# Grzetan/3D-Reconstruction-Triangulation

Hardware: NVIDIA B200
Metric: 3D points/sec (8-cam DLT, 20% missing) (higher is better)
Workload: dtype f64

## Files before the change

3d-reconstruction-triangulation_b200/csrc/tri_matrix.cu:

```cuda
#include "tri_pipe.cuh"

namespace tri {

__device__ __forceinline__ void load12(const double (&src)[12], double (&P)[12]) {
  const double2* v = reinterpret_cast<const double2*>(src);
#pragma unroll
  for (int k = 0; k < 6; k++) { const double2 q = v[k]; P[2 * k] = q.x; P[2 * k + 1] = q.y; }
}
__device__ __forceinline__ void load12(const float (&src)[12], float (&P)[12]) {
  const float4* v = reinterpret_cast<const float4*>(src);
#pragma unroll
  for (int k = 0; k < 3; k++) { const float4 q = v[k]; P[4 * k] = q.x; P[4 * k + 1] = q.y; P[4 * k + 2] = q.z; P[4 * k + 3] = q.w; }
}

template <typename T>
__device__ __forceinline__ void acc_row(T a0, T a1, T a2, T b, T (&M)[6], T (&v)[3]) {
  M[0] = fma_(a0, a0, M[0]); M[1] = fma_(a0, a1, M[1]); M[2] = fma_(a0, a2, M[2]); v[0] = fma_(a0, b, v[0]);
  M[3] = fma_(a1, a1, M[3]); M[4] = fma_(a1, a2, M[4]); v[1] = fma_(a1, b, v[1]);
  M[5] = fma_(a2, a2, M[5]); v[2] = fma_(a2, b, v[2]);
}

template <typename T>
__device__ __forceinline__ const T* absent_row(const DltRig<T>& rig, uint32_t mask, int group, int n_in_group) {
  const uint32_t absent = ~(mask >> (8 * group)) & ((1u << n_in_group) - 1u);
  return rig.absent + ((size_t)group * 256 + absent) * DLT_TABLE_ROW;
}
__device__ __forceinline__ void sub_row(const float* row, float (&M)[6], float (&v)[3]) {
  const float4* r = reinterpret_cast<const float4*>(row);
  const float4 t0 = __ldg(r), t1 = __ldg(r + 1), t2 = __ldg(r + 2);
  M[0] -= t0.x; M[1] -= t0.y; M[2] -= t0.z; M[3] -= t0.w; M[4] -= t1.x; M[5] -= t1.y; v[0] -= t1.z; v[1] -= t1.w; v[2] -= t2.x;
}

// ... 14 lines not shown
    T P[12];
    load12(rig.P[c], P);
    if constexpr (CENTRED) { x -= rig.pix0[c][0]; y -= rig.pix0[c][1]; }
    if constexpr (MASKING == MASK_TABLE) { x = valid ? x : T(0); y = valid ? y : T(0); }
#pragma unroll
    for (int r = 0; r < 2; r++) {
      const T u = r == 0 ? x : y;
      T a0 = fma_(-u, P[8], P[4 * r]), a1 = fma_(-u, P[9], P[4 * r + 1]), a2 = fma_(-u, P[10], P[4 * r + 2]);
      const T b = fma_(u, P[11], -P[4 * r + 3]);
      if constexpr (MASKING == MASK_SELECT_HI) { a0 = mask_coeff(a0, valid); a1 = mask_coeff(a1, valid); a2 = mask_coeff(a2, valid); }
      acc_row<T>(a0, a1, a2, b, a.M, a.v);
    }
  }
  static __device__ __forceinline__ void add_chunk(const Rig& rig, int c, T x, T y, bool valid, Acc& a) { add(rig, c, x, y, valid, a); }
  static __device__ __forceinline__ void solve(const Rig& rig, const Acc& a, uint32_t mask, int, T (&X)[3], int, int&) {
    Acc r = a;
    if constexpr (MASKING == MASK_TABLE)
      for (int g = 0; 8 * g < rig.n_use; g++) sub_row(absent_row<T>(rig, mask, g, min(8, rig.n_use - 8 * g)), r.M, r.v);
    solve_sym3<T>(r.M, r.v, X);
  }
  static __device__ __forceinline__ T residual(const Rig& rig, int c, T x, T y, const T (&X)[3]) {
    const T(&P)[12] = rig.P[c];
    if constexpr (CENTRED) { x -= rig.pix0[c][0]; y -= rig.pix0[c][1]; }
    const T e0 = fma_(fma_(-x, P[8], P[0]), X[0], fma_(fma_(-x, P[9], P[1]), X[1], fma_(fma_(-x, P[10], P[2]), X[2], -fma_(x, P[11], -P[3]))));
    const T e1 = fma_(fma_(-y, P[8], P[4]), X[0], fma_(fma_(-y, P[9], P[5]), X[1], fma_(fma_(-y, P[10], P[6]), X[2], -fma_(y, P[11], -P[7]))));
    return fma_(e0, e0, mul_(e1, e1));
  }
  static __device__ __forceinline__ double error(T sum, int n) { return sqrt((double)sum / (double)(2 * n)); }
  static __device__ __forceinline__ void to_world(const Rig& rig, T (&X)[3]) {
    if constexpr (CENTRED) { X[0] += rig.origin[0]; X[1] += rig.origin[1]; X[2] += rig.origin[2]; }
  }
};

struct DltTile64 {
  static constexpr int FPT = 2;
  using S = DltPolicy<double, false, MASK_SELECT_HI>;
  using Rig = DltRig<double>;
  using Real = double;
  template <int NC, int PIX, bool WIDE, class RS>
  static __device__ __forceinline__ void run(const Rig& rig, const RS& raw, int, double (&X)[2][3], uint32_t (&mask)[2],
                                             double (&err)[2], int (&iters)[2]) {
    typename S::Acc acc[2];
    mask[0] = mask[1] = 0;
#pragma unroll
    for (int c = 0; c < NC; c++) {
      double P[12];
      load12(rig.P[c], P);
      double x[2], y[2];
      bool ok[2];
      if constexpr (PIX == PIX_F32) {
        const Views<float, PIX, 2> q = decode<float, PIX, 2>(raw[c]);
#pragma unroll
        for (int j = 0; j < 2; j++) { ok[j] = q.v[j]; x[j] = (double)q.x[j]; y[j] = (double)q.y[j]; }
      } else {
        const Views<double, PIX, 2> q = decode<double, PIX, 2>(raw[c]);
#pragma unroll
        for (int j = 0; j < 2; j++) { ok[j] = q.v[j]; x[j] = q.x[j]; y[j] = q.y[j]; }
      }
#pragma unroll
      for (int j = 0; j < 2; j++) {
        mask[j] |= (ok[j] ? 1u : 0u) << c;
#pragma unroll
        for (int r = 0; r < 2; r++) {
          const double u = r == 0 ? x[j] : y[j];
          double a0 = fma_(-u, P[8], P[4 * r]), a1 = fma_(-u, P[9], P[4 * r + 1]), a2 = fma_(-u, P[10], P[4 * r + 2]);
          const double b = fma_(u, P[11], -P[4 * r + 3]);
          a0 = mask_coeff(a0, ok[j]); a1 = mask_coeff(a1, ok[j]); a2 = mask_coeff(a2, ok[j]);
          acc_row<double>(a0, a1, a2, b, acc[j].M, acc[j].v);
        }
      }
    }
#pragma unroll
    for (int j = 0; j < 2; j++) {
      X[j][0] = X[j][1] = X[j][2] = 0;
      err[j] = 0;
      iters[j] = 0;
      const int n = __popc(mask[j]);
      if (n >= 2) {
        solve_sym3<double>(acc[j].M, acc[j].v, X[j]);
        if constexpr (WIDE) {
          double e = 0;
#pragma unroll
          for (int c = 0; c < NC; c++) {
            const Views<double, PIX, 2> q = decode<double, PIX, 2>(raw[c]);
            if (q.v[j]) e += S::residual(rig, c, q.x[j], q.y[j], X[j]);
          }
          err[j] = S::error(e, n);
        }
      }
    }
  }
};

struct __align__(16) DltRigX2 {
  float2 A[TRI_MAX_CAMS][8];
  float2 N[TRI_MAX_CAMS][4];
  float2 npix0[TRI_MAX_CAMS][2];
  float origin[3];
  const float* absent;
};

struct DltX2Tile {
  static constexpr int FPT = 2;
  using Rig = DltRigX2;
  using Real = float;
  template <int NC, int PIX, bool WIDE, class RS>
  static __device__ __forceinline__ void run(const Rig& rig, const RS& raw, int, float (&X)[2][3], uint32_t (&mask)[2],
                                             double (&err)[2], int (&iters)[2]) {
    float2 M[6] = {{0, 0}, {0, 0}, {0, 0}, {0, 0}, {0, 0}, {0, 0}}, v[3] = {{0, 0}, {0, 0}, {0, 0}};
    uint32_t mask0 = 0, mask1 = 0;
#pragma unroll
    for (int c = 0; c < NC; c++) {
// ... 49 lines not shown
            if (q.v[j]) {
              const float x = q.x[j] + rig.npix0[c][0].x, y = q.y[j] + rig.npix0[c][1].x;
              const float e0 = fmaf(fmaf(x, rig.N[c][0].x, rig.A[c][0].x), Xr[j][0], fmaf(fmaf(x, rig.N[c][1].x, rig.A[c][1].x), Xr[j][1],
                               fmaf(fmaf(x, rig.N[c][2].x, rig.A[c][2].x), Xr[j][2], -fmaf(x, rig.N[c][3].x, rig.A[c][3].x))));
              const float e1 = fmaf(fmaf(y, rig.N[c][0].x, rig.A[c][4].x), Xr[j][0], fmaf(fmaf(y, rig.N[c][1].x, rig.A[c][5].x), Xr[j][1],
                               fmaf(fmaf(y, rig.N[c][2].x, rig.A[c][6].x), Xr[j][2], -fmaf(y, rig.N[c][3].x, rig.A[c][7].x))));
              e += fmaf(e0, e0, e1 * e1);
            }
          }
          err[j] = sqrt((double)e / (double)(2 * __popc(j == 0 ? mask0 : mask1)));
        }
      }
      X[j][0] = ok ? Xr[j][0] + rig.origin[0] : 0.f; X[j][1] = ok ? Xr[j][1] + rig.origin[1] : 0.f; X[j][2] = ok ? Xr[j][2] + rig.origin[2] : 0.f;
    }
  }
};


static DltRigX2 make_x2(const DltRig<float>& r) {
  DltRigX2 x;
  for (int c = 0; c < TRI_MAX_CAMS; c++) {
    const float* P = r.P[c];
    const float A[8] = {P[0], P[1], P[2], -P[3], P[4], P[5], P[6], -P[7]};
    const float N[4] = {-P[8], -P[9], -P[10], P[11]};
    for (int k = 0; k < 8; k++) x.A[c][k] = make_float2(A[k], A[k]);
    for (int k = 0; k < 4; k++) x.N[c][k] = make_float2(N[k], N[k]);
    for (int k = 0; k < 2; k++) x.npix0[c][k] = make_float2(-r.pix0[c][k], -r.pix0[c][k]);
  }
  for (int k = 0; k < 3; k++) x.origin[k] = r.origin[k];
  x.absent = r.absent;
  return x;
}

cudaError_t launch_dlt(const LaunchCtx& ctx, bool f32, int pixfmt, const DltRig<double>& rig64_,
                       const DltRig<float>& rig32_, const void* d_xy, int n_use, int64_t n_frames,
                       int64_t cam_stride, const BatchOut& out) {
  if (n_frames <= 0) return cudaSuccess;
  using P32 = DltPolicy<float, true, MASK_TABLE>;
  using P64 = DltPolicy<double, false, MASK_SELECT_HI>;
  if (f32) {
    DltRig<float> rig32 = rig32_;
    rig32.n_use = n_use;
    const DltRigX2 x2 = make_x2(rig32);
    if (pixfmt == PIX_F32) return launch_streamed<DltX2Tile, P32, PIX_F32, 2, 2, 3, true>(ctx, x2, rig32, d_xy, n_use, n_frames, cam_stride, out, 0);
    if (pixfmt == PIX_F64) return launch_streamed<DltX2Tile, P32, PIX_F64, 2, 2, 3>(ctx, x2, rig32, d_xy, n_use, n_frames, cam_stride, out, 0);
    return launch_streamed<DltX2Tile, P32, PIX_U16, 2, 2, 3>(ctx, x2, rig32, d_xy, n_use, n_frames, cam_stride, out, 0);
  }
  DltRig<double> rig64 = rig64_;
  rig64.n_use = n_use;
  if (pixfmt == PIX_F32) return launch_streamed<DltTile64, P64, PIX_F32, 2, 2, 2>(ctx, rig64, rig64, d_xy, n_use, n_frames, cam_stride, out, 0);
  if (pixfmt == PIX_F64) return launch_batch_policy<P64, PIX_F64, 1, 3>(ctx, rig64, d_xy, n_use, n_frames, cam_stride, out, 0);
  return launch_streamed<DltTile64, P64, PIX_U16, 2, 3, 2>(ctx, rig64, rig64, d_xy, n_use, n_frames, cam_stride, out, 0);
}

}
```

3d-reconstruction-triangulation_b200/csrc/tri_api.cu:

```cuda
#include <math.h>
#include <stdlib.h>
#include <string.h>

#include <algorithm>
#include <string>
#include <thread>
#include <vector>

#include "tri_engine.cuh"

namespace tri {

static thread_local std::string g_error;
void set_error(const std::string& s) { g_error = s; }
int fail(int status, const std::string& s) {
  g_error = s;
  return status;
}
int cuda_fail(cudaError_t err, const char* what) {
  g_error = std::string(what) + ": " + cudaGetErrorString(err);
  return TRI_ERR_CUDA;
}
#define TRI_CUDA(call)                                         \
  do {                                                         \
// ... 90 lines not shown
static cudaError_t upload_ray_table(RayFold<T>& f, int n_cams) {
  const std::vector<T> tab = ray_mask_table(f, n_cams);
  T* d = nullptr;
  cudaError_t err = cudaMalloc((void**)&d, tab.size() * sizeof(T));
  if (err == cudaSuccess) err = cudaMemcpy(d, tab.data(), tab.size() * sizeof(T), cudaMemcpyHostToDevice);
  f.mask_table = d;
  return err;
}

static inline float fma_h(float a, float b, float c) { return fmaf(a, b, c); }
template <typename T>
static std::vector<T> dlt_absent_table(const DltRig<T>& r, int n_cams) {
  const int groups = (n_cams + 7) / 8;
  std::vector<T> tab((size_t)groups * 256 * DLT_TABLE_ROW, (T)0);
  for (int g = 0; g < groups; g++)
    for (int m = 0; m < 256; m++) {
      T M[6] = {0, 0, 0, 0, 0, 0}, v[3] = {0, 0, 0};
      for (int k = 0; k < 8 && 8 * g + k < n_cams; k++) {
        if (!(m >> k & 1)) continue;
        const T* P = r.P[8 * g + k];
        for (int row = 0; row < 2; row++) {
          const T a0 = P[4 * row], a1 = P[4 * row + 1], a2 = P[4 * row + 2], b = -P[4 * row + 3];
          M[0] = fma_h(a0, a0, M[0]); M[1] = fma_h(a0, a1, M[1]); M[2] = fma_h(a0, a2, M[2]); v[0] = fma_h(a0, b, v[0]);
          M[3] = fma_h(a1, a1, M[3]); M[4] = fma_h(a1, a2, M[4]); v[1] = fma_h(a1, b, v[1]);
          M[5] = fma_h(a2, a2, M[5]); v[2] = fma_h(a2, b, v[2]);
        }
      }
      T* row = &tab[((size_t)g * 256 + m) * DLT_TABLE_ROW];
      for (int k = 0; k < 6; k++) row[k] = M[k];
      for (int k = 0; k < 3; k++) row[6 + k] = v[k];
    }
  return tab;
}
template <typename T>
static cudaError_t upload_dlt_table(DltRig<T>& r, int n_cams) {
  const std::vector<T> tab = dlt_absent_table(r, n_cams);
  T* d = nullptr;
  cudaError_t err = cudaMalloc((void**)&d, tab.size() * sizeof(T));
  if (err == cudaSuccess) err = cudaMemcpy(d, tab.data(), tab.size() * sizeof(T), cudaMemcpyHostToDevice);
  r.absent = d;
  return err;
}

static void build_rigs(tri_engine* e) {
  memset(&e->fold64, 0, sizeof(e->fold64));
  memset(&e->fold32, 0, sizeof(e->fold32));
  memset(&e->rig64, 0, sizeof(e->rig64));
  memset(&e->rig32, 0, sizeof(e->rig32));
  memset(&e->ray, 0, sizeof(e->ray));
  double c0[3];
  rig_centre(e, c0);
  for (int k = 0; k < 3; k++) e->rig32.origin[k] = (float)c0[k];
  for (int k = 0; k < 3; k++) c0[k] = (double)e->rig32.origin[k];
  for (int c = 0; c < e->n_cams; c++) {
    const tri_camera& cam = e->cams[c];
    for (int k = 0; k < 12; k++) e->rig64.P[c][k] = cam.P[k];
    const double px = floor(cam.width / 2.0), py = floor(cam.height / 2.0);
    double Q[12];
    for (int k = 0; k < 4; k++) {
      Q[k] = cam.P[k] - px * cam.P[8 + k];
      Q[4 + k] = cam.P[4 + k] - py * cam.P[8 + k];
      Q[8 + k] = cam.P[8 + k];
    }
    for (int r = 0; r < 3; r++) Q[r * 4 + 3] += Q[r * 4] * c0[0] + Q[r * 4 + 1] * c0[1] + Q[r * 4 + 2] * c0[2];
    for (int k = 0; k < 12; k++) e->rig32.P[c][k] = (float)Q[k];
    e->rig32.pix0[c][0] = (float)px;
    e->rig32.pix0[c][1] = (float)py;
    e->ray.aspect[c] = (double)cam.width / (double)cam.height;
    e->ray.width[c] = (double)cam.width;
// ... 157 lines not shown
int tri_version(void) { return 100; }
const char* tri_last_error(void) { return g_error.c_str(); }

int tri_device_count(void) {
  int n = 0;
  if (cudaGetDeviceCount(&n) != cudaSuccess) {
    cudaGetLastError();
    return 0;
  }
  return n;
}

int tri_create(int n_cams, const tri_camera* cams, int device, tri_engine** out) {
  if (!out) return fail(TRI_ERR_ARG, "null out pointer");
  *out = nullptr;
  if (n_cams < 1 || n_cams > TRI_MAX_CAMS || !cams) return fail(TRI_ERR_ARG, "n_cams must be in [1, TRI_MAX_CAMS]");
  int n_dev = tri_device_count();
  if (n_dev <= 0) return fail(TRI_ERR_NO_DEVICE, "no CUDA device: the engine has no CPU path");
  if (device < 0 || device >= n_dev) return fail(TRI_ERR_ARG, "device index out of range");
  for (int c = 0; c < n_cams; c++)
    if (cams[c].width <= 0 || cams[c].height <= 0) return fail(TRI_ERR_ARG, "camera width/height must be positive");
  DeviceGuard g(device);
  cudaDeviceProp prop;
  TRI_CUDA(cudaGetDeviceProperties(&prop, device));
  if (prop.major < 10) return fail(TRI_ERR_NO_DEVICE, "libtri_b200 is built for sm_100a (B200) only");
  tri_engine* e = new tri_engine();
  e->device = device;
  e->n_cams = n_cams;
  e->sm_count = prop.multiProcessorCount;
  memcpy(e->cams, cams, sizeof(tri_camera) * n_cams);
  build_rigs(e);
  cudaError_t err = cudaMalloc((void**)&e->d_first_bad, 2 * sizeof(unsigned long long));
  if (err == cudaSuccess) err = cudaMemset(e->d_first_bad, 0xff, 2 * sizeof(unsigned long long));
  if (err == cudaSuccess) err = upload_dlt_table(e->rig32, n_cams);
  if (err == cudaSuccess) err = upload_ray_table(e->fold64, n_cams);
  if (err == cudaSuccess) err = upload_ray_table(e->fold32, n_cams);
  if (err == cudaSuccess) err = cudaStreamCreateWithFlags(&e->stream, cudaStreamNonBlocking);
  for (int i = 0; i < N_SLOTS && err == cudaSuccess; i++) err = cudaStreamCreateWithFlags(&e->slots[i].stream, cudaStreamNonBlocking);
  if (err != cudaSuccess) {
    int st = cuda_fail(err, "tri_create");
    tri_destroy(e);
    return st;
  }
  *out = e;
  return TRI_OK;
}

void tri_destroy(tri_engine* e) {
  if (!e) return;
  DeviceGuard g(e->device);
  cudaDeviceSynchronize();
  for (int i = 0; i < N_SLOTS; i++) {
    if (e->slots[i].d_in) cudaFree(e->slots[i].d_in);
    if (e->slots[i].d_out) cudaFree(e->slots[i].d_out);
    if (e->slots[i].stream) cudaStreamDestroy(e->slots[i].stream);
  }
  if (e->cls_work && e->cls_work_free) e->cls_work_free(e->cls_work);
  if (e->d_scratch) cudaFree(e->d_scratch);
  if (e->stream) cudaStreamDestroy(e->stream);
  if (e->d_first_bad) cudaFree(e->d_first_bad);
  if (e->rig32.absent) cudaFree(const_cast<float*>(e->rig32.absent));
  if (e->fold64.mask_table) cudaFree(const_cast<double*>(e->fold64.mask_table));
  if (e->fold32.mask_table) cudaFree(const_cast<float*>(e->fold32.mask_table));
  delete e;
}

int tri_engine_device(const tri_engine* e) { return e ? e->device : -1; }
int tri_engine_cameras(const tri_engine* e) { return e ? e->n_cams : 0; }
int64_t tri_kernel_launches(const tri_engine* e) { return e ? e->launches : 0; }

int tri_triangulate_points_device(tri_engine* e, int mode, unsigned flags, const void* d_xy, int n_point_cams,
                                  int64_t n_frames, int64_t cam_stride, const tri_batch_out* d_out, void* stream) {
  int n_use = 0, fmt = 0;
  int st = check_batch_args(e, mode, d_xy, n_point_cams, n_frames, cam_stride, d_out, &n_use);
  if (st != TRI_OK) return st;
  if ((st = pix_format(flags, &fmt)) != TRI_OK) return st;
  if (n_frames == 0) return TRI_OK;
  DeviceGuard g(e->device);
  BatchOut out{d_out->xyz_f32, d_out->xyz_f64, d_out->mask, d_out->err, d_out->iters};
  if (n_use == 0) return too_few_device(e, n_frames, out, (cudaStream_t)stream);
  return launch_batch(e, e->ctx((cudaStream_t)stream), mode, flags, fmt, d_xy, n_use, n_frames, cam_stride, out);
}

int tri_enable_peer_access(tri_engine* e, int peer_device) {
  if (!e) return fail(TRI_ERR_ARG, "null engine");
  if (peer_device == e->device) return TRI_OK;
  DeviceGuard g(e->device);
  int can = 0;
  TRI_CUDA(cudaDeviceCanAccessPeer(&can, e->device, peer_device));
  if (!can) return fail(TRI_ERR_ARG, "no peer access between these GPUs");
  cudaError_t err = cudaDeviceEnablePeerAccess(peer_device, 0);
  if (err == cudaErrorPeerAccessAlreadyEnabled) { cudaGetLastError(); return TRI_OK; }
  if (err != cudaSuccess) return cuda_fail(err, "cudaDeviceEnablePeerAccess");
  return TRI_OK;
// ... 182 lines not shown
```

3d-reconstruction-triangulation_b200/csrc/tri_batch.cuh:

```cuda
#pragma once
#include "tri_common.cuh"

namespace tri {

constexpr int BATCH_THREADS = 256;

template <typename T>
struct View2 {
  T x0, y0, x1, y1;
  bool v0, v1;
};

template <typename T, int PIX>
__device__ __forceinline__ View2<T> fetch2(const char* row, int64_t pair) {
  View2<T> r;
  if constexpr (PIX == PIX_F32) {
    float4 q = ld_stream(reinterpret_cast<const float4*>(row) + pair);
    r.v0 = pix_valid(q.x, q.y);
    r.v1 = pix_valid(q.z, q.w);
    r.x0 = to_real<T>(q.x); r.y0 = to_real<T>(q.y); r.x1 = to_real<T>(q.z); r.y1 = to_real<T>(q.w);
  } else if constexpr (PIX == PIX_F64) {
    double2 a = ld_stream(reinterpret_cast<const double2*>(row) + 2 * pair);
    double2 b = ld_stream(reinterpret_cast<const double2*>(row) + 2 * pair + 1);
    r.v0 = pix_valid(a.x, a.y);
    r.v1 = pix_valid(b.x, b.y);
    r.x0 = (T)a.x; r.y0 = (T)a.y; r.x1 = (T)b.x; r.y1 = (T)b.y;
  } else {
    uint2 q = ld_stream(reinterpret_cast<const uint2*>(row) + pair);
    r.v0 = q.x != 0xffffffffu;
    r.v1 = q.y != 0xffffffffu;
    if constexpr (sizeof(T) == 8) {
      const double magic = 4503599627370496.0;
      r.x0 = __hiloint2double(0x43300000, (int)(q.x & 0xffffu)) - magic;
// ... 9 lines not shown

template <typename T, int PIX>
__device__ __forceinline__ void fetch1(const char* row, int64_t f, T& x, T& y, bool& v) {
  if constexpr (PIX == PIX_F32) {
    float2 q = ld_stream(reinterpret_cast<const float2*>(row) + f);
    v = pix_valid(q.x, q.y); x = (T)q.x; y = (T)q.y;
  } else if constexpr (PIX == PIX_F64) {
    double2 q = ld_stream(reinterpret_cast<const double2*>(row) + f);
    v = pix_valid(q.x, q.y); x = (T)q.x; y = (T)q.y;
  } else {
    unsigned q = ld_stream(reinterpret_cast<const unsigned*>(row) + f);
    v = q != 0xffffffffu; x = (T)(q & 0xffffu); y = (T)(q >> 16);
  }
}

template <typename T, int PIX, int FPT>
struct Views {
  T x[FPT], y[FPT];
  bool v[FPT];
};

template <typename T, int PIX, int FPT>
__device__ __forceinline__ Views<T, PIX, FPT> fetch(const char* row, int64_t group) {
  Views<T, PIX, FPT> r;
  if constexpr (FPT == 2) {
    View2<T> w = fetch2<T, PIX>(row, group);
    r.x[0] = w.x0; r.y[0] = w.y0; r.v[0] = w.v0; r.x[1] = w.x1; r.y[1] = w.y1; r.v[1] = w.v1;
  } else {
    fetch1<T, PIX>(row, group, r.x[0], r.y[0], r.v[0]);
  }
  return r;
}

template <class S, int NC, int PIX, int FPT, int MINB>
__global__ void __launch_bounds__(BATCH_THREADS, MINB)
batch_kernel(const __grid_constant__ typename S::Rig rig, const char* __restrict__ xy, int64_t row_bytes,
             int64_t n_groups, int n_use, BatchOut out, int opt, unsigned long long* first_bad, int64_t frame_base) {
  using T = typename S::T;
  __shared__ __align__(16) float tile[BATCH_THREADS * 3 * FPT];
  const int64_t block_group0 = (int64_t)blockIdx.x * BATCH_THREADS;
  const int64_t group = block_group0 + threadIdx.x;
  const int nc = NC > 0 ? NC : n_use;
  T X[FPT][3];
#pragma unroll
  for (int j = 0; j < FPT; j++) X[j][0] = X[j][1] = X[j][2] = 0;

  if (group < n_groups) {
    typename S::Acc acc[FPT];
    uint32_t mask[FPT];
    T e[FPT];
    int it[FPT], n[FPT];
#pragma unroll
    for (int j = 0; j < FPT; j++) { mask[j] = 0; e[j] = 0; it[j] = 0; }
    if constexpr (NC > 0) {
      Views<T, PIX, FPT> w[NC];
#pragma unroll
      for (int c = 0; c < NC; c++) w[c] = fetch<T, PIX, FPT>(xy + c * row_bytes, group);
#pragma unroll
      for (int c = 0; c < NC; c++)
#pragma unroll
        for (int j = 0; j < FPT; j++)
          { S::add(rig, c, w[c].x[j], w[c].y[j], w[c].v[j], acc[j]); mask[j] |= (w[c].v[j] ? 1u : 0u) << c; }
#pragma unroll
      for (int j = 0; j < FPT; j++) {
        n[j] = __popc(mask[j]);
        if (n[j] >= 2) S::solve(rig, acc[j], mask[j], n[j], X[j], opt, it[j]);
      }
      if (out.err) {
#pragma unroll
        for (int c = 0; c < NC; c++)
#pragma unroll
          for (int j = 0; j < FPT; j++)
            if (w[c].v[j]) e[j] += S::residual(rig, c, w[c].x[j], w[c].y[j], X[j]);
      }
    } else {
#pragma unroll 4
      for (int c = 0; c < nc; c++) {
        Views<T, PIX, FPT> w = fetch<T, PIX, FPT>(xy + c * row_bytes, group);
#pragma unroll
        for (int j = 0; j < FPT; j++)
          { S::add(rig, c, w.x[j], w.y[j], w.v[j], acc[j]); mask[j] |= (w.v[j] ? 1u : 0u) << c; }
      }
#pragma unroll
      for (int j = 0; j < FPT; j++) {
        n[j] = __popc(mask[j]);
        if (n[j] >= 2) S::solve(rig, acc[j], mask[j], n[j], X[j], opt, it[j]);
      }
      if (out.err) {
        for (int c = 0; c < nc; c++) {
          Views<T, PIX, FPT> w = fetch<T, PIX, FPT>(xy + c * row_bytes, group);
#pragma unroll
          for (int j = 0; j < FPT; j++)
            if (w.v[j]) e[j] += S::residual(rig, c, w.x[j], w.y[j], X[j]);
        }
      }
    }
#pragma unroll
    for (int j = 0; j < FPT; j++) {
      const int64_t f = FPT * group + j;
      if (n[j] >= 2) S::to_world(rig, X[j]);
      else atomicMin(first_bad, (unsigned long long)(frame_base + f));
      if (out.xyz_f64) { double* o = out.xyz_f64 + 3 * f; o[0] = X[j][0]; o[1] = X[j][1]; o[2] = X[j][2]; }
      if (out.mask) out.mask[f] = mask[j];
      if (out.err) out.err[f] = n[j] >= 2 ? S::error(e[j], n[j]) : 0.0;
      if (out.iters) out.iters[f] = it[j];
    }
  }

  if (out.xyz_f32) {
    float* t = tile + 3 * FPT * threadIdx.x;
#pragma unroll
    for (int j = 0; j < FPT; j++) { t[3 * j] = (float)X[j][0]; t[3 * j + 1] = (float)X[j][1]; t[3 * j + 2] = (float)X[j][2]; }
    __syncthreads();
    const int64_t remaining = n_groups - block_group0;
    float* dst = out.xyz_f32 + 3 * FPT * block_group0;
    if (remaining >= BATCH_THREADS && ((uintptr_t)dst & 15) == 0) {
      float4* d4 = reinterpret_cast<float4*>(dst);
      const float4* s4 = reinterpret_cast<const float4*>(tile);
#pragma unroll
      for (int i = threadIdx.x; i < BATCH_THREADS * 3 * FPT / 4; i += BATCH_THREADS) __stcs(d4 + i, s4[i]);
    } else {
      const int cnt = (int)(remaining < BATCH_THREADS ? remaining : BATCH_THREADS) * 3 * FPT;
      for (int i = threadIdx.x; i < cnt; i += BATCH_THREADS) dst[i] = tile[i];
    }
  }
}

template <class S, int PIX>
__global__ void __launch_bounds__(BATCH_THREADS)
batch_single_kernel(const __grid_constant__ typename S::Rig rig, const char* __restrict__ xy, int64_t row_bytes,
                    int64_t f_begin, int64_t f_end, int n_use, BatchOut out, int opt, unsigned long long* first_bad,
                    int64_t frame_base) {
  using T = typename S::T;
  const int64_t f = f_begin + (int64_t)blockIdx.x * BATCH_THREADS + threadIdx.x;
  if (f >= f_end) return;
  typename S::Acc acc;
  T X[3] = {0, 0, 0}, e = 0;
  uint32_t mask = 0;
  int it = 0;
  for (int c = 0; c < n_use; c++) {
    T x, y; bool ok;
    fetch1<T, PIX>(xy + c * row_bytes, f, x, y, ok);
    { S::add(rig, c, x, y, ok, acc); mask |= (ok ? 1u : 0u) << c; }
  }
  const int n = __popc(mask);
  if (n >= 2) {
    S::solve(rig, acc, mask, n, X, opt, it);
    if (out.err)
      for (int c = 0; c < n_use; c++) {
        T x, y; bool ok;
        fetch1<T, PIX>(xy + c * row_bytes, f, x, y, ok);
        if (ok) e += S::residual(rig, c, x, y, X);
      }
    S::to_world(rig, X);
  } else {
    atomicMin(first_bad, (unsigned long long)(frame_base + f));
  }
  if (out.xyz_f32) { float* o = out.xyz_f32 + 3 * f; o[0] = (float)X[0]; o[1] = (float)X[1]; o[2] = (float)X[2]; }
  if (out.xyz_f64) { double* o = out.xyz_f64 + 3 * f; o[0] = X[0]; o[1] = X[1]; o[2] = X[2]; }
  if (out.mask) out.mask[f] = mask;
  if (out.err) out.err[f] = n >= 2 ? S::error(e, n) : 0.0;
  if (out.iters) out.iters[f] = it;
}

template <class S, int PIX, int FPT, int MINB>
static cudaError_t launch_batch_policy(const LaunchCtx& ctx, const typename S::Rig& rig, const void* d_xy, int n_use,
                                       int64_t n_frames, int64_t cam_stride, const BatchOut& out, int opt) {
  const char* xy = static_cast<const char*>(d_xy);
  const int64_t row_bytes = cam_stride * pix_bytes(PIX);
  const int64_t need = FPT * pix_bytes(PIX);
  const bool vec = FPT == 1 || (((uintptr_t)xy % need == 0) && (row_bytes % need == 0));
  const int64_t n_groups = vec ? n_frames / FPT : 0;
  if (n_groups > 0) {
    const unsigned grid = (unsigned)((n_groups + BATCH_THREADS - 1) / BATCH_THREADS);
#define TRI_CASE(N)                                                                                              \
  case N:                                                                                                        \
    batch_kernel<S, N, PIX, FPT, MINB><<<grid, BATCH_THREADS, 0, ctx.stream>>>(rig, xy, row_bytes, n_groups, n_use, \
                                                                               out, opt, ctx.d_first_bad,        \
                                                                               ctx.frame_base);                  \
    break;
// ... 21 lines not shown
```

3d-reconstruction-triangulation_b200/csrc/tri_common.cuh:

```cuda
#pragma once
#include <cuda_runtime.h>
#include <stdint.h>

#include "../../include/tri_b200.h"

namespace tri {


constexpr int DLT_TABLE_ROW = 12;
template <typename T>
struct __align__(16) DltRig {
  T P[TRI_MAX_CAMS][12];
  T pix0[TRI_MAX_CAMS][2];
  T origin[3];
  const T* absent;
  int n_use;
};

struct RayRig {
  double aspect[TRI_MAX_CAMS];
  double width[TRI_MAX_CAMS], height[TRI_MAX_CAMS];
  double depth[TRI_MAX_CAMS];
  double quat[TRI_MAX_CAMS][4];
  double pos[TRI_MAX_CAMS][3];
};

template <typename T>
struct __align__(16) RayFold {
  T U0[TRI_MAX_CAMS][3], U1[TRI_MAX_CAMS][3], U2[TRI_MAX_CAMS][3];
  T ax[TRI_MAX_CAMS], bx[TRI_MAX_CAMS], ay[TRI_MAX_CAMS], by[TRI_MAX_CAMS], dd[TRI_MAX_CAMS];
  T n4[TRI_MAX_CAMS];
  T ob[TRI_MAX_CAMS][3];
  T n4ob[TRI_MAX_CAMS][3];
  T n4ob2[TRI_MAX_CAMS];
  T origin[3];
  const T* mask_table;
};
constexpr int TRI_RAY_TABLE_CAMS = 8;

struct BatchOut {
  float* xyz_f32;
  double* xyz_f64;
  uint32_t* mask;
  double* err;
  int32_t* iters;
};

enum PixFmt { PIX_F32 = 0, PIX_F64 = 1, PIX_U16 = 2 };

__host__ __device__ inline int pix_bytes(int fmt) { return fmt == PIX_F32 ? 8 : fmt == PIX_F64 ? 16 : 4; }
// ... 79 lines not shown
```

3d-reconstruction-triangulation_b200/csrc/tri_pipe.cuh:

```cuda
#pragma once
#include <type_traits>

#include "tri_batch.cuh"

namespace tri {

__device__ __forceinline__ uint32_t smem_u32(const void* p) { return (uint32_t)__cvta_generic_to_shared(p); }

template <int PIX, int FPT> struct RawPix;
template <> struct RawPix<PIX_F32, 2> { using type = float4; };
template <> struct RawPix<PIX_F32, 1> { using type = float2; };
template <> struct RawPix<PIX_U16, 2> { using type = uint2; };
template <> struct RawPix<PIX_U16, 1> { using type = unsigned; };

template <typename T, int PIX, int FPT>
__device__ __forceinline__ Views<T, PIX, FPT> decode(const typename RawPix<PIX, FPT>::type& q) {
  Views<T, PIX, FPT> r;
  if constexpr (PIX == PIX_F32 && FPT == 2) {
    r.v[0] = pix_valid(q.x, q.y); r.v[1] = pix_valid(q.z, q.w);
    r.x[0] = to_real<T>(q.x); r.y[0] = to_real<T>(q.y); r.x[1] = to_real<T>(q.z); r.y[1] = to_real<T>(q.w);
  } else if constexpr (PIX == PIX_F32 && FPT == 1) {
    r.v[0] = pix_valid(q.x, q.y); r.x[0] = to_real<T>(q.x); r.y[0] = to_real<T>(q.y);
  } else if constexpr (PIX == PIX_U16 && FPT == 2) {
    r.v[0] = q.x != 0xffffffffu; r.v[1] = q.y != 0xffffffffu;
// ... 347 lines not shown
    cudaError_t err = cudaFuncSetAttribute(kern, cudaFuncAttributeMaxDynamicSharedMemorySize, bytes);
    if (err != cudaSuccess) return err;
    int per_sm = 1;
    err = cudaOccupancyMaxActiveBlocksPerMultiprocessor(&per_sm, kern, BATCH_THREADS, bytes);
    if (err != cudaSuccess) return err;
    const int64_t grid = std::min<int64_t>(n_tiles, (int64_t)ctx.sm_count * std::max(per_sm, 1));
    kern<<<(unsigned)grid, BATCH_THREADS, bytes, ctx.stream>>>(rig, xy, row_bytes, n_tiles, n_use, out, opt, ctx.d_first_bad, ctx.frame_base);
    return cudaGetLastError();
  };
  const cudaError_t err = wants_wide(out) ? go(chunk_kernel<S, PIX, FPT, STAGES, MINB, true>) : go(chunk_kernel<S, PIX, FPT, STAGES, MINB, false>);
  if (err != cudaSuccess) return err;
  ++*ctx.launches;
  *covered = n_tiles * TILE;
  return cudaSuccess;
}

inline BatchOut advance(const BatchOut& o, int64_t frames) {
  BatchOut r = o;
  if (r.xyz_f32) r.xyz_f32 += 3 * frames;
  if (r.xyz_f64) r.xyz_f64 += 3 * frames;
  if (r.mask) r.mask += frames;
  if (r.err) r.err += frames;
  if (r.iters) r.iters += frames;
  return r;
}


template <class TS, class S, int PIX, int FPT, int STAGES, int MINB, bool LAZY = false>
static cudaError_t launch_streamed(const LaunchCtx& ctx, const typename TS::Rig& tile_rig, const typename S::Rig& rig,
                                   const void* d_xy, int n_use, int64_t n_frames, int64_t cam_stride, const BatchOut& out, int opt) {
  int64_t covered = 0;
  if constexpr (PIX != PIX_F64) {
    cudaError_t err;
    if (S::CHUNKED && n_use > CHUNK_CAMS)
      err = launch_chunk<S, PIX, S::CHUNK_FPT, 3, 2>(ctx, rig, d_xy, n_use, n_frames, cam_stride, out, opt, &covered);
    else
      err = launch_stream<TS, PIX, STAGES, MINB, LAZY>(ctx, tile_rig, d_xy, n_use, n_frames, cam_stride, out, opt, &covered);
    if (err != cudaSuccess || covered == n_frames) return err;
  }
  LaunchCtx rest = ctx;
  rest.frame_base += covered;
  return launch_batch_policy<S, PIX, FPT, (MINB > 3 ? 3 : MINB)>(rest, rig, static_cast<const char*>(d_xy) + covered * pix_bytes(PIX), n_use,
                                                n_frames - covered, cam_stride, advance(out, covered), opt);
}

}
```

Baseline: 53.65 billion.

## Replace f32-to-f64 pixel conversion with bit-shift construction and prescaled camera rows

For f32 pixels in the f64 DLT tile, each float is turned into a double by shifting its bits directly, which yields the value scaled by 2^-896. The last projection row is prescaled by 2^896 on the host so the products come out unchanged. A max-abs check with NaN propagation catches inf/NaN inputs and falls back to a noinline path that uses ordinary conversions. The aim is to avoid the F2F conversion instructions, whose f64 throughput is limited. The risks are wrong handling of denormal pixels and an extra argument passed to launch_streamed.

```diff
diff --git a/3d-reconstruction-triangulation_b200/csrc/tri_matrix.cu b/3d-reconstruction-triangulation_b200/csrc/tri_matrix.cu
--- a/3d-reconstruction-triangulation_b200/csrc/tri_matrix.cu
+++ b/3d-reconstruction-triangulation_b200/csrc/tri_matrix.cu
@@ -1,3 +1,5 @@
+#include <cmath>
+
 #include "tri_pipe.cuh"
 
 namespace tri {
@@ -78,26 +80,53 @@
   }
 };
 
+struct DltRigTile64 {
+  DltRig<double> rig;
+  double N[TRI_MAX_CAMS][4];
+  int scaled;
+};
+
+__device__ __forceinline__ double f32_scaled(float x) {
+  const int b = __float_as_int(x);
+  return __hiloint2double((b >> 3) & (int)0x8fffffff, (int)((unsigned)b << 29));
+}
+__device__ __forceinline__ float max_abs_nan(float m, float x) {
+  float r;
+  asm("max.NaN.f32 %0, %1, %2;" : "=f"(r) : "f"(m), "f"(fabsf(x)));
+  return r;
+}
+
 struct DltTile64 {
   static constexpr int FPT = 2;
   using S = DltPolicy<double, false, MASK_SELECT_HI>;
-  using Rig = DltRig<double>;
+  using Rig = DltRigTile64;
   using Real = double;
-  template <int NC, int PIX, bool WIDE, class RS>
-  static __device__ __forceinline__ void run(const Rig& rig, const RS& raw, int, double (&X)[2][3], uint32_t (&mask)[2],
-                                             double (&err)[2], int (&iters)[2]) {
-    typename S::Acc acc[2];
-    mask[0] = mask[1] = 0;
+
+  template <int NC, int PIX, bool SCALED, class RS>
+  static __device__ __forceinline__ bool accumulate(const Rig& rt, const RS& raw, typename S::Acc (&acc)[2], uint32_t (&mask)[2]) {
+    const DltRig<double>& rig = rt.rig;
+    float big = 0.f;
+#pragma unroll
+    for (int j = 0; j < 2; j++) { acc[j] = typename S::Acc(); mask[j] = 0; }
 #pragma unroll
     for (int c = 0; c < NC; c++) {
       double P[12];
       load12(rig.P[c], P);
+      if constexpr (SCALED) { P[8] = rt.N[c][0]; P[9] = rt.N[c][1]; P[10] = rt.N[c][2]; P[11] = rt.N[c][3]; }
       double x[2], y[2];
       bool ok[2];
       if constexpr (PIX == PIX_F32) {
         const Views<float, PIX, 2> q = decode<float, PIX, 2>(raw[c]);
 #pragma unroll
-        for (int j = 0; j < 2; j++) { ok[j] = q.v[j]; x[j] = (double)q.x[j]; y[j] = (double)q.y[j]; }
+        for (int j = 0; j < 2; j++) {
+          ok[j] = q.v[j];
+          if constexpr (SCALED) {
+            x[j] = f32_scaled(q.x[j]); y[j] = f32_scaled(q.y[j]);
+            big = max_abs_nan(max_abs_nan(big, q.x[j]), q.y[j]);
+          } else {
+            x[j] = (double)q.x[j]; y[j] = (double)q.y[j];
+          }
+        }
       } else {
         const Views<double, PIX, 2> q = decode<double, PIX, 2>(raw[c]);
 #pragma unroll
@@ -115,6 +144,34 @@
           acc_row<double>(a0, a1, a2, b, acc[j].M, acc[j].v);
         }
       }
+    }
+    return !SCALED || big <= 3.402823466e38f;
+  }
+
+  struct Sums {
+    typename S::Acc acc[2];
+    uint32_t mask[2];
+  };
+  template <int NC, int PIX, class RS>
+  static __device__ __noinline__ Sums accumulate_f2f(const Rig& rt, const RS raw) {
+    Sums s;
+    accumulate<NC, PIX, false>(rt, raw, s.acc, s.mask);
+    return s;
+  }
+
+  template <int NC, int PIX, bool WIDE, class RS>
+  static __device__ __forceinline__ void run(const Rig& rt, const RS& raw, int, double (&X)[2][3], uint32_t (&mask)[2],
+                                             double (&err)[2], int (&iters)[2]) {
+    const DltRig<double>& rig = rt.rig;
+    typename S::Acc acc[2];
+    if constexpr (PIX == PIX_F32) {
+      if (!rt.scaled || !accumulate<NC, PIX, true>(rt, raw, acc, mask)) {
+        const Sums s = accumulate_f2f<NC, PIX>(rt, raw);
+#pragma unroll
+        for (int j = 0; j < 2; j++) { acc[j] = s.acc[j]; mask[j] = s.mask[j]; }
+      }
+    } else {
+      accumulate<NC, PIX, false>(rt, raw, acc, mask);
     }
 #pragma unroll
     for (int j = 0; j < 2; j++) {
@@ -239,6 +296,18 @@
   return x;
 }
 
+static DltRigTile64 make_tile64(const DltRig<double>& r) {
+  DltRigTile64 t;
+  t.rig = r;
+  t.scaled = 1;
+  for (int c = 0; c < TRI_MAX_CAMS; c++)
+    for (int k = 0; k < 4; k++) {
+      t.N[c][k] = std::ldexp(r.P[c][8 + k], 896);
+      if (!std::isfinite(t.N[c][k])) t.scaled = 0;
+    }
+  return t;
+}
+
 cudaError_t launch_dlt(const LaunchCtx& ctx, bool f32, int pixfmt, const DltRig<double>& rig64_,
                        const DltRig<float>& rig32_, const void* d_xy, int n_use, int64_t n_frames,
                        int64_t cam_stride, const BatchOut& out) {
@@ -255,9 +324,10 @@
   }
   DltRig<double> rig64 = rig64_;
   rig64.n_use = n_use;
-  if (pixfmt == PIX_F32) return launch_streamed<DltTile64, P64, PIX_F32, 2, 2, 2>(ctx, rig64, rig64, d_xy, n_use, n_frames, cam_stride, out, 0);
   if (pixfmt == PIX_F64) return launch_batch_policy<P64, PIX_F64, 1, 3>(ctx, rig64, d_xy, n_use, n_frames, cam_stride, out, 0);
-  return launch_streamed<DltTile64, P64, PIX_U16, 2, 3, 2>(ctx, rig64, rig64, d_xy, n_use, n_frames, cam_stride, out, 0);
-}
-
-}
+  const DltRigTile64 t64 = make_tile64(rig64);
+  if (pixfmt == PIX_F32) return launch_streamed<DltTile64, P64, PIX_F32, 2, 2, 2, true>(ctx, t64, rig64, d_xy, n_use, n_frames, cam_stride, out, 0);
+  return launch_streamed<DltTile64, P64, PIX_U16, 2, 3, 2>(ctx, t64, rig64, d_xy, n_use, n_frames, cam_stride, out, 0);
+}
+
+}
```

Measured after the change: 50.59 billion (median of 6 runs). 5.7% lower.

## Precompute per-camera DLT moment coefficients and mask base table for f64 path

Applied to the files above, without the earlier changes.

The f64 DLT path now expands the normal-equation accumulation algebraically. Each camera contributes a constant part, looked up from a 256-entry table indexed by the validity mask, plus terms linear in x, y and x²+y² with precomputed moment coefficients K. The per-camera projection-row arithmetic is replaced by 27 FMAs against constants held in the grid-constant rig. Invalid views are zeroed instead of masked. This cuts per-point FLOPs but enlarges the kernel parameter struct, adds a global table load per point, and may shift rounding slightly.

```diff
diff --git a/3d-reconstruction-triangulation_b200/csrc/tri_api.cu b/3d-reconstruction-triangulation_b200/csrc/tri_api.cu
--- a/3d-reconstruction-triangulation_b200/csrc/tri_api.cu
+++ b/3d-reconstruction-triangulation_b200/csrc/tri_api.cu
@@ -146,9 +146,21 @@
     }
   return tab;
 }
+static std::vector<double> dlt_base_table(const DltRig<double>& r, int n_cams) {
+  std::vector<double> tab((size_t)256 * DLT_TABLE_ROW, 0.0);
+  for (int m = 0; m < 256; m++) {
+    double* row = &tab[(size_t)m * DLT_TABLE_ROW];
+    for (int c = 0; c < 8 && c < n_cams; c++) {
+      if (!(m >> c & 1)) continue;
+      double K[DLT_MOMENTS], K0D0[9];
+      dlt_moments(r.P[c], K, K0D0);
+      for (int i = 0; i < 9; i++) row[i] += K0D0[i];
+    }
+  }
+  return tab;
+}
 template <typename T>
-static cudaError_t upload_dlt_table(DltRig<T>& r, int n_cams) {
-  const std::vector<T> tab = dlt_absent_table(r, n_cams);
+static cudaError_t upload_dlt_table(DltRig<T>& r, const std::vector<T>& tab) {
   T* d = nullptr;
   cudaError_t err = cudaMalloc((void**)&d, tab.size() * sizeof(T));
   if (err == cudaSuccess) err = cudaMemcpy(d, tab.data(), tab.size() * sizeof(T), cudaMemcpyHostToDevice);
@@ -372,7 +384,8 @@
   build_rigs(e);
   cudaError_t err = cudaMalloc((void**)&e->d_first_bad, 2 * sizeof(unsigned long long));
   if (err == cudaSuccess) err = cudaMemset(e->d_first_bad, 0xff, 2 * sizeof(unsigned long long));
-  if (err == cudaSuccess) err = upload_dlt_table(e->rig32, n_cams);
+  if (err == cudaSuccess) err = upload_dlt_table(e->rig32, dlt_absent_table(e->rig32, n_cams));
+  if (err == cudaSuccess) err = upload_dlt_table(e->rig64, dlt_base_table(e->rig64, n_cams));
   if (err == cudaSuccess) err = upload_ray_table(e->fold64, n_cams);
   if (err == cudaSuccess) err = upload_ray_table(e->fold32, n_cams);
   if (err == cudaSuccess) err = cudaStreamCreateWithFlags(&e->stream, cudaStreamNonBlocking);
@@ -400,6 +413,7 @@
   if (e->stream) cudaStreamDestroy(e->stream);
   if (e->d_first_bad) cudaFree(e->d_first_bad);
   if (e->rig32.absent) cudaFree(const_cast<float*>(e->rig32.absent));
+  if (e->rig64.absent) cudaFree(const_cast<double*>(e->rig64.absent));
   if (e->fold64.mask_table) cudaFree(const_cast<double*>(e->fold64.mask_table));
   if (e->fold32.mask_table) cudaFree(const_cast<float*>(e->fold32.mask_table));
   delete e;
diff --git a/3d-reconstruction-triangulation_b200/csrc/tri_batch.cuh b/3d-reconstruction-triangulation_b200/csrc/tri_batch.cuh
--- a/3d-reconstruction-triangulation_b200/csrc/tri_batch.cuh
+++ b/3d-reconstruction-triangulation_b200/csrc/tri_batch.cuh
@@ -1,4 +1,6 @@
 #pragma once
+#include <type_traits>
+
 #include "tri_common.cuh"
 
 namespace tri {
@@ -74,6 +76,28 @@
   return r;
 }
 
+template <class S, class = void>
+struct HasBegin { static constexpr bool value = false; };
+template <class S>
+struct HasBegin<S, std::void_t<decltype(S::BEGIN)>> { static constexpr bool value = S::BEGIN; };
+
+template <class S, int PIX, int FPT>
+__device__ __forceinline__ void begin_views(const typename S::Rig& rig, const char* xy, int64_t row_bytes, int64_t group, int nc,
+                                            typename S::Acc (&acc)[FPT]) {
+  if constexpr (HasBegin<S>::value) {
+    uint32_t bits[FPT];
+#pragma unroll
+    for (int j = 0; j < FPT; j++) bits[j] = 0;
+    for (int c = 0; c < nc; c++) {
+      const Views<typename S::T, PIX, FPT> w = fetch<typename S::T, PIX, FPT>(xy + c * row_bytes, group);
+#pragma unroll
+      for (int j = 0; j < FPT; j++) bits[j] |= (w.v[j] ? 1u : 0u) << c;
+    }
+#pragma unroll
+    for (int j = 0; j < FPT; j++) S::begin(rig, bits[j], acc[j]);
+  }
+}
+
 template <class S, int NC, int PIX, int FPT, int MINB>
 __global__ void __launch_bounds__(BATCH_THREADS, MINB)
 batch_kernel(const __grid_constant__ typename S::Rig rig, const char* __restrict__ xy, int64_t row_bytes,
@@ -98,6 +122,15 @@
       Views<T, PIX, FPT> w[NC];
 #pragma unroll
       for (int c = 0; c < NC; c++) w[c] = fetch<T, PIX, FPT>(xy + c * row_bytes, group);
+      if constexpr (HasBegin<S>::value) {
+#pragma unroll
+        for (int j = 0; j < FPT; j++) {
+          uint32_t bits = 0;
+#pragma unroll
+          for (int c = 0; c < NC; c++) bits |= (w[c].v[j] ? 1u : 0u) << c;
+          S::begin(rig, bits, acc[j]);
+        }
+      }
 #pragma unroll
       for (int c = 0; c < NC; c++)
 #pragma unroll
@@ -116,6 +149,7 @@
             if (w[c].v[j]) e[j] += S::residual(rig, c, w[c].x[j], w[c].y[j], X[j]);
       }
     } else {
+      begin_views<S, PIX, FPT>(rig, xy, row_bytes, group, nc, acc);
 #pragma unroll 4
       for (int c = 0; c < nc; c++) {
         Views<T, PIX, FPT> w = fetch<T, PIX, FPT>(xy + c * row_bytes, group);
@@ -176,18 +210,19 @@
   using T = typename S::T;
   const int64_t f = f_begin + (int64_t)blockIdx.x * BATCH_THREADS + threadIdx.x;
   if (f >= f_end) return;
-  typename S::Acc acc;
+  typename S::Acc acc[1];
   T X[3] = {0, 0, 0}, e = 0;
   uint32_t mask = 0;
   int it = 0;
+  begin_views<S, PIX, 1>(rig, xy, row_bytes, f, n_use, acc);
   for (int c = 0; c < n_use; c++) {
     T x, y; bool ok;
     fetch1<T, PIX>(xy + c * row_bytes, f, x, y, ok);
-    { S::add(rig, c, x, y, ok, acc); mask |= (ok ? 1u : 0u) << c; }
+    { S::add(rig, c, x, y, ok, acc[0]); mask |= (ok ? 1u : 0u) << c; }
   }
   const int n = __popc(mask);
   if (n >= 2) {
-    S::solve(rig, acc, mask, n, X, opt, it);
+    S::solve(rig, acc[0], mask, n, X, opt, it);
     if (out.err)
       for (int c = 0; c < n_use; c++) {
         T x, y; bool ok;
diff --git a/3d-reconstruction-triangulation_b200/csrc/tri_common.cuh b/3d-reconstruction-triangulation_b200/csrc/tri_common.cuh
--- a/3d-reconstruction-triangulation_b200/csrc/tri_common.cuh
+++ b/3d-reconstruction-triangulation_b200/csrc/tri_common.cuh
@@ -16,6 +16,26 @@
   const T* absent;
   int n_use;
 };
+
+constexpr int DLT_MOMENTS = 28;
+inline void dlt_moments(const double P[12], double K[DLT_MOMENTS], double K0D0[9]) {
+  static const int I[6] = {0, 0, 0, 1, 1, 2}, J[6] = {0, 1, 2, 1, 2, 2};
+  const double *p0 = P, *p1 = P + 4, *q = P + 8;
+  for (int k = 0; k < 6; k++) {
+    const int i = I[k], j = J[k];
+    K0D0[k] = fma(p0[i], p0[j], p1[i] * p1[j]);
+    K[3 * k] = -fma(p0[i], q[j], q[i] * p0[j]);
+    K[3 * k + 1] = -fma(p1[i], q[j], q[i] * p1[j]);
+    K[3 * k + 2] = q[i] * q[j];
+  }
+  for (int i = 0; i < 3; i++) {
+    K0D0[6 + i] = -fma(P[3], p0[i], P[7] * p1[i]);
+    K[18 + 3 * i] = fma(P[11], p0[i], P[3] * q[i]);
+    K[18 + 3 * i + 1] = fma(P[11], p1[i], P[7] * q[i]);
+    K[18 + 3 * i + 2] = -(P[11] * q[i]);
+  }
+  K[27] = 0;
+}
 
 struct RayRig {
   double aspect[TRI_MAX_CAMS];
diff --git a/3d-reconstruction-triangulation_b200/csrc/tri_matrix.cu b/3d-reconstruction-triangulation_b200/csrc/tri_matrix.cu
--- a/3d-reconstruction-triangulation_b200/csrc/tri_matrix.cu
+++ b/3d-reconstruction-triangulation_b200/csrc/tri_matrix.cu
@@ -78,43 +78,84 @@
   }
 };
 
+struct __align__(16) DltRig64 {
+  DltRig<double> d;
+  double K[8][DLT_MOMENTS];
+};
+
+__device__ __forceinline__ void load_row(const double* row, double (&M)[6], double (&v)[3]) {
+  const double2* r = reinterpret_cast<const double2*>(row);
+  const double2 t0 = __ldg(r), t1 = __ldg(r + 1), t2 = __ldg(r + 2), t3 = __ldg(r + 3), t4 = __ldg(r + 4);
+  M[0] = t0.x; M[1] = t0.y; M[2] = t1.x; M[3] = t1.y; M[4] = t2.x; M[5] = t2.y; v[0] = t3.x; v[1] = t3.y; v[2] = t4.x;
+}
+
+__device__ __forceinline__ void add_moments(const double (&K)[DLT_MOMENTS], double x, double y, double (&M)[6], double (&v)[3]) {
+  const double s = fma_(x, x, mul_(y, y));
+#pragma unroll
+  for (int k = 0; k < 6; k++) { M[k] = fma_(x, K[3 * k], M[k]); M[k] = fma_(y, K[3 * k + 1], M[k]); M[k] = fma_(s, K[3 * k + 2], M[k]); }
+#pragma unroll
+  for (int i = 0; i < 3; i++) { v[i] = fma_(x, K[18 + 3 * i], v[i]); v[i] = fma_(y, K[18 + 3 * i + 1], v[i]); v[i] = fma_(s, K[18 + 3 * i + 2], v[i]); }
+}
+
+struct DltPolicy64 {
+  using T = double;
+  using Rig = DltRig64;
+  static constexpr bool CHUNKED = false;
+  static constexpr bool BEGIN = true;
+  struct Acc {
+    T M[6] = {0, 0, 0, 0, 0, 0};
+    T v[3] = {0, 0, 0};
+  };
+  static __device__ __forceinline__ void begin(const Rig& rig, uint32_t bits, Acc& a) {
+    load_row(rig.d.absent + (size_t)bits * DLT_TABLE_ROW, a.M, a.v);
+  }
+  static __device__ __forceinline__ void add(const Rig& rig, int c, T x, T y, bool valid, Acc& a) {
+    add_moments(rig.K[c], valid ? x : 0.0, valid ? y : 0.0, a.M, a.v);
+  }
+  static __device__ __forceinline__ void solve(const Rig&, const Acc& a, uint32_t, int, T (&X)[3], int, int&) { solve_sym3<T>(a.M, a.v, X); }
+  static __device__ __forceinline__ T residual(const Rig& rig, int c, T x, T y, const T (&X)[3]) {
+    const T(&P)[12] = rig.d.P[c];
+    const T e0 = fma_(fma_(-x, P[8], P[0]), X[0], fma_(fma_(-x, P[9], P[1]), X[1], fma_(fma_(-x, P[10], P[2]), X[2], -fma_(x, P[11], -P[3]))));
+    const T e1 = fma_(fma_(-y, P[8], P[4]), X[0], fma_(fma_(-y, P[9], P[5]), X[1], fma_(fma_(-y, P[10], P[6]), X[2], -fma_(y, P[11], -P[7]))));
+    return fma_(e0, e0, mul_(e1, e1));
+  }
+  static __device__ __forceinline__ double error(T sum, int n) { return sqrt(sum / (double)(2 * n)); }
+  static __device__ __forceinline__ void to_world(const Rig&, T (&)[3]) {}
+};
+
+__device__ __forceinline__ Views<double, PIX_F32, 2> decode_zeroed(float4 q) {
+  if (!pix_valid(q.x, q.y)) q.x = q.y = 0.f;
+  if (!pix_valid(q.z, q.w)) q.z = q.w = 0.f;
+  return decode<double, PIX_F32, 2>(q);
+}
+__device__ __forceinline__ Views<double, PIX_U16, 2> decode_zeroed(uint2 q) {
+  return decode<double, PIX_U16, 2>(make_uint2(q.x != 0xffffffffu ? q.x : 0u, q.y != 0xffffffffu ? q.y : 0u));
+}
+
 struct DltTile64 {
   static constexpr int FPT = 2;
-  using S = DltPolicy<double, false, MASK_SELECT_HI>;
-  using Rig = DltRig<double>;
+  using S = DltPolicy64;
+  using Rig = DltRig64;
   using Real = double;
   template <int NC, int PIX, bool WIDE, class RS>
   static __device__ __forceinline__ void run(const Rig& rig, const RS& raw, int, double (&X)[2][3], uint32_t (&mask)[2],
                                              double (&err)[2], int (&iters)[2]) {
-    typename S::Acc acc[2];
     mask[0] = mask[1] = 0;
 #pragma unroll
     for (int c = 0; c < NC; c++) {
-      double P[12];
-      load12(rig.P[c], P);
-      double x[2], y[2];
-      bool ok[2];
-      if constexpr (PIX == PIX_F32) {
-        const Views<float, PIX, 2> q = decode<float, PIX, 2>(raw[c]);
-#pragma unroll
-        for (int j = 0; j < 2; j++) { ok[j] = q.v[j]; x[j] = (double)q.x[j]; y[j] = (double)q.y[j]; }
-      } else {
-        const Views<double, PIX, 2> q = decode<double, PIX, 2>(raw[c]);
-#pragma unroll
-        for (int j = 0; j < 2; j++) { ok[j] = q.v[j]; x[j] = q.x[j]; y[j] = q.y[j]; }
-      }
-#pragma unroll
-      for (int j = 0; j < 2; j++) {
-        mask[j] |= (ok[j] ? 1u : 0u) << c;
-#pragma unroll
-        for (int r = 0; r < 2; r++) {
-          const double u = r == 0 ? x[j] : y[j];
-          double a0 = fma_(-u, P[8], P[4 * r]), a1 = fma_(-u, P[9], P[4 * r + 1]), a2 = fma_(-u, P[10], P[4 * r + 2]);
-          const double b = fma_(u, P[11], -P[4 * r + 3]);
-          a0 = mask_coeff(a0, ok[j]); a1 = mask_coeff(a1, ok[j]); a2 = mask_coeff(a2, ok[j]);
-          acc_row<double>(a0, a1, a2, b, acc[j].M, acc[j].v);
-        }
-      }
+      const Views<float, PIX, 2> q = decode<float, PIX, 2>(raw[c]);
+      mask[0] |= (q.v[0] ? 1u : 0u) << c;
+      mask[1] |= (q.v[1] ? 1u : 0u) << c;
+    }
+    double M[2][6], v[2][3];
+#pragma unroll
+    for (int j = 0; j < 2; j++) load_row(rig.d.absent + (size_t)mask[j] * DLT_TABLE_ROW, M[j], v[j]);
+    constexpr int UNROLL = NC > 2 ? 8 : 1;
+#pragma unroll UNROLL
+    for (int c = 0; c < NC; c++) {
+      const Views<double, PIX, 2> q = decode_zeroed(raw[c]);
+#pragma unroll
+      for (int j = 0; j < 2; j++) add_moments(rig.K[c], q.x[j], q.y[j], M[j], v[j]);
     }
 #pragma unroll
     for (int j = 0; j < 2; j++) {
@@ -123,7 +164,7 @@
       iters[j] = 0;
       const int n = __popc(mask[j]);
       if (n >= 2) {
-        solve_sym3<double>(acc[j].M, acc[j].v, X[j]);
+        solve_sym3<double>(M[j], v[j], X[j]);
         if constexpr (WIDE) {
           double e = 0;
 #pragma unroll
@@ -253,11 +294,24 @@
     if (pixfmt == PIX_F64) return launch_streamed<DltX2Tile, P32, PIX_F64, 2, 2, 3>(ctx, x2, rig32, d_xy, n_use, n_frames, cam_stride, out, 0);
     return launch_streamed<DltX2Tile, P32, PIX_U16, 2, 2, 3>(ctx, x2, rig32, d_xy, n_use, n_frames, cam_stride, out, 0);
   }
-  DltRig<double> rig64 = rig64_;
-  rig64.n_use = n_use;
-  if (pixfmt == PIX_F32) return launch_streamed<DltTile64, P64, PIX_F32, 2, 2, 2>(ctx, rig64, rig64, d_xy, n_use, n_frames, cam_stride, out, 0);
-  if (pixfmt == PIX_F64) return launch_batch_policy<P64, PIX_F64, 1, 3>(ctx, rig64, d_xy, n_use, n_frames, cam_stride, out, 0);
-  return launch_streamed<DltTile64, P64, PIX_U16, 2, 3, 2>(ctx, rig64, rig64, d_xy, n_use, n_frames, cam_stride, out, 0);
-}
-
-}
+  if (n_use > 8) {
+    DltRig<double> rig64 = rig64_;
+    rig64.n_use = n_use;
+    if (pixfmt == PIX_F32) return launch_batch_policy<P64, PIX_F32, 2, 2>(ctx, rig64, d_xy, n_use, n_frames, cam_stride, out, 0);
+    if (pixfmt == PIX_F64) return launch_batch_policy<P64, PIX_F64, 1, 3>(ctx, rig64, d_xy, n_use, n_frames, cam_stride, out, 0);
+    return launch_batch_policy<P64, PIX_U16, 2, 2>(ctx, rig64, d_xy, n_use, n_frames, cam_stride, out, 0);
+  }
+  DltRig64 rig64;
+  rig64.d = rig64_;
+  rig64.d.n_use = n_use;
+  for (int c = 0; c < 8; c++) {
+    double K0D0[9];
+    dlt_moments(rig64.d.P[c], rig64.K[c], K0D0);
+  }
+  using M64 = DltPolicy64;
+  if (pixfmt == PIX_F32) return launch_streamed<DltTile64, M64, PIX_F32, 2, 2, 2, true>(ctx, rig64, rig64, d_xy, n_use, n_frames, cam_stride, out, 0);
+  if (pixfmt == PIX_F64) return launch_batch_policy<M64, PIX_F64, 1, 3>(ctx, rig64, d_xy, n_use, n_frames, cam_stride, out, 0);
+  return launch_streamed<DltTile64, M64, PIX_U16, 2, 3, 2, true>(ctx, rig64, rig64, d_xy, n_use, n_frames, cam_stride, out, 0);
+}
+
+}
diff --git a/3d-reconstruction-triangulation_b200/csrc/tri_pipe.cuh b/3d-reconstruction-triangulation_b200/csrc/tri_pipe.cuh
--- a/3d-reconstruction-triangulation_b200/csrc/tri_pipe.cuh
+++ b/3d-reconstruction-triangulation_b200/csrc/tri_pipe.cuh
@@ -403,10 +403,14 @@
   int64_t covered = 0;
   if constexpr (PIX != PIX_F64) {
     cudaError_t err;
-    if (S::CHUNKED && n_use > CHUNK_CAMS)
-      err = launch_chunk<S, PIX, S::CHUNK_FPT, 3, 2>(ctx, rig, d_xy, n_use, n_frames, cam_stride, out, opt, &covered);
-    else
+    if constexpr (S::CHUNKED) {
+      if (n_use > CHUNK_CAMS)
+        err = launch_chunk<S, PIX, S::CHUNK_FPT, 3, 2>(ctx, rig, d_xy, n_use, n_frames, cam_stride, out, opt, &covered);
+      else
+        err = launch_stream<TS, PIX, STAGES, MINB, LAZY>(ctx, tile_rig, d_xy, n_use, n_frames, cam_stride, out, opt, &covered);
+    } else {
       err = launch_stream<TS, PIX, STAGES, MINB, LAZY>(ctx, tile_rig, d_xy, n_use, n_frames, cam_stride, out, opt, &covered);
+    }
     if (err != cudaSuccess || covered == n_frames) return err;
   }
   LaunchCtx rest = ctx;
```

Result: slower. 53.46 billion before, 42.73 billion after, median of 6 (-20.1%).
